# schwanbeck/YSMR

Measured on AMD Instinct MI355X. Metric: frames/sec detect+link, 1228x922 ~500 blobs, 1/2/4/8 GPU; HBM GB/s %peak, higher is better.
Workload: dtype u8 image / f32 threshold+geometry / f64 link; 1 GPU; 1228x922 stream, ~500 blobs, detect+link end to end (BASELINE configs[2], the configuration the metric is quoted on); detect_batch=248, channels=1, streams=1, parallelism=1 stream/GPU x1, tracks_alive=508, ids_issued=796

## Files before the change

ysmr_amd/csrc/detect_plan.h:

```cpp
#pragma once
#include <algorithm>
#include <cmath>
#include <cstddef>
#include <cstdint>

#include "hd.h"
#include "ysmr_hip.h"

namespace detect_plan {

constexpr int CU_COUNT = 256;
constexpr int TW = 64, TH = 32;
constexpr int STRIP_HALO_LANES = 3;
constexpr int STRIP_MAX_OUT_LANES = 64 - 2 * STRIP_HALO_LANES;
constexpr int STRIP_RESIDENT = 768;
#ifndef TM_MAX_PANEL_N
#define TM_MAX_PANEL_N 1232
#endif
#ifndef TM_START_ROWS_N
#define TM_START_ROWS_N 48
#endif
constexpr int TM_START_ROWS = TM_START_ROWS_N;
constexpr int TM_MAX_PANEL = TM_MAX_PANEL_N;

constexpr int NR_STRIDE = 32;
constexpr int SHARED_COUNTERS = 8;
constexpr int HOLED_CAP = 4096;
constexpr int WIN_CORE = 32;
#ifndef WIN_GROUP_N
#define WIN_GROUP_N 8
#endif
constexpr int WIN_GROUP = WIN_GROUP_N;
constexpr int CLEAR_BLOCKS = 512;
#ifndef WINDOW_BLOCKS_N
#define WINDOW_BLOCKS_N 1024
#endif
constexpr int WINDOW_BLOCKS = WINDOW_BLOCKS_N;
#ifndef WINDOW_BLOCKS_FREE_N
// ... 87 lines not shown
    return (cv_flavour & YSMR_BESIDE_BATCH_LINK) ? 248 : ((cv_flavour & YSMR_BESIDE_SPLIT_LINK) ? 160 : CU_COUNT);
}

inline bool mfma_supported(int H, int W, int channels, int t_low, int t_high, int use_high)
{
    const int gap = use_high ? (t_high > t_low ? t_high - t_low : t_low - t_high) : 1;
    return channels == 1 && (W & 3) == 0 && W >= 64 && W <= 16384 && H >= 18 && H <= 16383 && gap >= 1 &&
           t_low > -1000 && t_low < 1000 && t_high > -1000 && t_high < 1000;
}

struct StripShape {
    int out_lanes, strips_x, seg_h, segs_y;
    int by_xcd;
    unsigned blocks;
};
struct MfmaShape {
    int panels, panel_w;
    int by_xcd;
    int start_rows;
    unsigned grid;
};
enum class Kernel { refused, mfma, strip, tile };
struct ThresholdPlan {
    Kernel kernel;
    int mfma_variant;
    MfmaShape mfma;
    StripShape strip;
    unsigned tile_grid[3];
};

inline MfmaShape mfma_shape(int batch, int H, int W, int blocks_wanted, size_t mfma_lds)
{
    MfmaShape m{};
    m.panels = (W + TM_MAX_PANEL - 1) / TM_MAX_PANEL;
    m.panel_w = ((W + m.panels - 1) / m.panels + 15) & ~15;
    m.panels = (W + m.panel_w - 1) / m.panel_w;
    const int per_cu = (int)((160 * 1024) / mfma_lds);
    const int blocks = blocks_wanted * per_cu;
    const long long grid = std::max<long long>(1, std::min<long long>((long long)batch * m.panels * H / 32, blocks));
    m.by_xcd = (batch % 8 == 0 && grid % 8 == 0) ? 1 : 0;
    const long long groups = m.by_xcd ? 8 : 1, cols = (long long)(batch / groups) * m.panels, nb = grid / groups;
    m.start_rows = nb % cols == 0 ? 0 : TM_START_ROWS;
    m.grid = (unsigned)grid;
    return m;
}

inline StripShape strip_shape(int batch, int H, int W, const Knobs &kn)
{
    StripShape s{};
    const int quads = (W + 3) / 4;
    s.strips_x = (quads + STRIP_MAX_OUT_LANES - 1) / STRIP_MAX_OUT_LANES;
    s.out_lanes = (quads + s.strips_x - 1) / s.strips_x;
    const int resident = kn.thr_blocks > 0 ? kn.thr_blocks : STRIP_RESIDENT;
    const long long columns = (long long)batch * s.strips_x;
    const long long segs = std::max<long long>(1, (long long)resident * 4 / columns);
    s.seg_h = kn.seg_h > 0 ? kn.seg_h : (int)std::max<long long>(32, (H + segs - 1) / segs);
    s.segs_y = (H + s.seg_h - 1) / s.seg_h;
    const long long waves = columns * s.segs_y;
    long long blocks = std::min<long long>((waves + 3) / 4, resident);
    s.by_xcd = (batch % 8 == 0 && blocks % 8 == 0) ? 1 : 0;
    if (s.by_xcd && blocks / 8 * 4 > (long long)(batch / 8) * s.strips_x * s.segs_y)
        blocks = (((long long)(batch / 8) * s.strips_x * s.segs_y + 3) / 4) * 8;
    s.blocks = (unsigned)blocks;
    return s;
}

inline ThresholdPlan threshold_plan(int batch, int H, int W, int channels, int t_low, int t_high, int use_high, int cv_flavour,
                                    int variant, const Knobs &kn, size_t mfma_lds)
{
    ThresholdPlan p{};
    if (variant == 0 && (cv_flavour & YSMR_BESIDE_LINK)) variant = 1;
    if (variant != 1 && mfma_supported(H, W, channels, t_low, t_high, use_high)) {
        p.kernel = Kernel::mfma;
        p.mfma_variant = variant >= 2 ? variant - 1 : 0;
        p.mfma = mfma_shape(batch, H, W, kn.thr_blocks > 0 ? kn.thr_blocks : threshold_workgroups(cv_flavour), mfma_lds);
        return p;
    }
    if (variant >= 2) return p;
    const int t_gap = use_high ? (t_high > t_low ? t_high - t_low : t_low - t_high) : 0;
    if ((W & 3) == 0 && W >= 16 && H >= 2 && t_low > -100000 && t_low < 100000 && t_high > -100000 && t_high < 100000 && t_gap <= 127) {
        p.kernel = Kernel::strip;
        p.strip = strip_shape(batch, H, W, kn);
    } else {
        p.kernel = Kernel::tile;
        p.tile_grid[0] = (unsigned)((W + TW - 1) / TW); p.tile_grid[1] = (unsigned)((H + TH - 1) / TH); p.tile_grid[2] = (unsigned)batch;
    }
    return p;
// ... 151 lines not shown
```

ysmr_amd/csrc/thr_mfma.h:

```cpp
#pragma once
#include <hip/hip_runtime.h>
#include <cstdint>
#include "detect_plan.h"

namespace ysmr_thr {

struct Params {
    int H, W, batch;
    int panels, panel_w;
    int by_xcd;
    int inv, use_high, t_low, t_high;
    float neg_x_mul, k_first, d2;
    float col_scale, row_scale;
    uint32_t sh1, k1, sh2, k2;
    int start_rows;
    float kw[6];
};

size_t lds_bytes();

int launch(hipStream_t st, const uint8_t *frames, uint8_t *cls, int batch, int H, int W, int inv, int t_low, int t_high,
           int use_high, const float *gauss11, const detect_plan::MfmaShape &shape, int variant, hipEvent_t ev_start = nullptr,
           hipEvent_t ev_stop = nullptr);

}
```

ysmr_amd/csrc/thr_mfma.hip:

```cpp
#include "common.h"
#include "thr_mfma.h"
#include <cstring>
#include <mutex>
#include <type_traits>

namespace {

typedef _Float16 half8_t __attribute__((ext_vector_type(8)));
typedef _Float16 half2_t __attribute__((ext_vector_type(2)));
typedef float f32x4 __attribute__((ext_vector_type(4)));
typedef int i32x4 __attribute__((ext_vector_type(4)));
typedef uint32_t u32x4 __attribute__((ext_vector_type(4)));

#ifndef TM_MEM_WAVE_N
#define TM_MEM_WAVE_N 0
#endif
constexpr bool TM_MEM_WAVE = TM_MEM_WAVE_N != 0;
#ifndef TM_WAVES_N
#define TM_WAVES_N 16
#endif
constexpr int TM_WAVES = TM_WAVES_N, TM_THREADS = 64 * TM_WAVES;
constexpr int TM_ROWS = 16;
using detect_plan::TM_MAX_PANEL;
constexpr int TM_MAX_TILES = TM_MAX_PANEL / 16;
// ... 27 lines not shown
#define TM_STORE_AT_START_N 1
#endif
constexpr bool TM_STORE_AT_START = TM_STORE_AT_START_N != 0;
#ifndef TM_BLUR_GROUP_N
#define TM_BLUR_GROUP_N 1
#endif
constexpr int TM_BLUR_GROUP = TM_BLUR_GROUP_N;
#ifndef TM_PREFETCH_N
#define TM_PREFETCH_N 1
#endif
constexpr bool TM_PREFETCH = TM_PREFETCH_N != 0;
#ifndef TM_LIST_CAP_N
#define TM_LIST_CAP_N 248
#endif
constexpr int TM_LIST_CAP = TM_LIST_CAP_N;

#ifdef YSMR_STAMPS
constexpr int TM_ST_STEPS = 20, TM_ST_N = 8;
__device__ unsigned long long g_tm_stamps[TM_WAVES][TM_ST_STEPS][TM_ST_N];
#define TMSTAMP(step, k) do { if (blockIdx.x == TM_ST_BLOCK && (step) < TM_ST_STEPS && lane == 0) g_tm_stamps[wave][step][k] = __builtin_amdgcn_s_memtime(); } while (0)
#ifndef TM_ST_BLOCK
#define TM_ST_BLOCK 100
#endif
#else
#define TMSTAMP(step, k) do {} while (0)
#endif

__device__ __forceinline__ int opaque_lane(int lane) { asm volatile("" : "+v"(lane)); return lane; }

struct ThrItem {
    int f, x0, x1, y0, y1;
};

__device__ __forceinline__ int reflect101(int i, int n) { if (i < 0) i = -i; if (i >= n) i = 2 * (n - 1) - i; return i; }
__device__ __forceinline__ int clampi(int v, int lo, int hi) { return v < lo ? lo : (v > hi ? hi : v); }

__device__ __forceinline__ float sub_f16_lo(float x, uint32_t h)
{
    float r;
    asm("v_fma_mix_f32 %0, %1, -1.0, %2 op_sel_hi:[1,0,0]" : "=v"(r) : "v"(h), "v"(x));
    return r;
}
__device__ __forceinline__ float sub_f16_hi(float x, uint32_t h)
{
    float r;
    asm("v_fma_mix_f32 %0, %1, -1.0, %2 op_sel:[1,0,0] op_sel_hi:[1,0,0]" : "=v"(r) : "v"(h), "v"(x));
    return r;
// ... 46 lines not shown
    __builtin_amdgcn_wave_barrier();
    __builtin_amdgcn_fence(__ATOMIC_ACQUIRE, "wavefront");
    const int yy = clampi(y - 5 + min(dy, 10), 0, H - 1);
    const int ra = reflect101(yy - 1, H) - (y - 6), rb = yy - (y - 6), rc = reflect101(yy + 1, H) - (y - 6);
    float acc = 0.0f;
    uint32_t centre = 0;
#pragma unroll 1
    for (int i = 0; i < 11; ++i) {
        const int xx = clampi(x - 5 + i, 0, W - 1);
        const int ca = reflect101(xx - 1, W) - (x - 6), cb = xx - (x - 6), cc = reflect101(xx + 1, W) - (x - 6);
        const uint32_t s = win[16 * ra + ca] + 2u * win[16 * ra + cb] + win[16 * ra + cc] +
                           2u * (win[16 * rb + ca] + 2u * win[16 * rb + cb] + win[16 * rb + cc]) +
                           win[16 * rc + ca] + 2u * win[16 * rc + cb] + win[16 * rc + cc];
        const uint32_t b = (s + 8u) >> 4;
        if (i == 5) centre = b;
        acc = __builtin_fmaf((float)b, tap_weight(P, i), acc);
    }
    float m = __builtin_fmaf(__shfl(acc, base + 5, 64), P.kw[5], 0.0f);
#pragma unroll 1
    for (int j = 1; j <= 5; ++j) m = __builtin_fmaf(__shfl(acc, base + 5 + j, 64) + __shfl(acc, base + 5 - j, 64), P.kw[5 - j], m);
    const uint32_t s = (uint32_t)__shfl((int)centre, base + 5, 64);
    const int mi = clampi((int)__builtin_rintf(m), 0, 255);
    const int d = (int)s - mi;
    const int lo = P.inv ? (d <= P.t_low) : (d > P.t_low);
    const int hi = P.use_high ? (P.inv ? (d <= P.t_high) : (d > P.t_high)) : lo;
    return (uint32_t)(lo | (hi << 1));
}

__device__ __forceinline__ uint32_t exact_class_wave(const uint8_t *frame, const ysmr_thr::Params &P, int y, int x, int lane, uint8_t *scratch)
{
    const int H = P.H, W = P.W;
    uint8_t *win = scratch;
    float *bl = reinterpret_cast<float *>(scratch + 208);
    uint8_t g[3];
#pragma unroll
// ... 18 lines not shown
        const uint32_t sum = win[16 * ra + ca] + 2u * win[16 * ra + cb] + win[16 * ra + cc] +
                             2u * (win[16 * rb + ca] + 2u * win[16 * rb + cb] + win[16 * rb + cc]) +
                             win[16 * rc + ca] + 2u * win[16 * rc + cb] + win[16 * rc + cc];
        bl[12 * dy + i] = (float)((sum + 8u) >> 4);
    }
    __builtin_amdgcn_fence(__ATOMIC_RELEASE, "wavefront");
    __builtin_amdgcn_wave_barrier();
    __builtin_amdgcn_fence(__ATOMIC_ACQUIRE, "wavefront");
    const float *row = bl + 12 * min(lane, 10);
    float v[11];
#pragma unroll
    for (int i = 0; i < 11; ++i) v[i] = row[i];
    const float centre = bl[12 * 5 + 5];
    float acc = 0.0f;
#pragma unroll
    for (int i = 0; i < 11; ++i) acc = __builtin_fmaf(v[i], tap_weight(P, i), acc);
    auto at = [&](int l) { return __builtin_bit_cast(float, __builtin_amdgcn_readlane(__builtin_bit_cast(int, acc), l)); };
    float m = __builtin_fmaf(at(5), P.kw[5], 0.0f);
#pragma unroll
    for (int j = 1; j <= 5; ++j) m = __builtin_fmaf(at(5 + j) + at(5 - j), P.kw[5 - j], m);
    const int mi = clampi((int)__builtin_rintf(m), 0, 255);
    const int d = (int)centre - mi;
    const int lo = P.inv ? (d <= P.t_low) : (d > P.t_low);
    const int hi = P.use_high ? (P.inv ? (d <= P.t_high) : (d > P.t_high)) : lo;
    return (uint32_t)(lo | (hi << 1));
}

struct Lds {
    _Float16 tile[TM_PLANES ? 4 * TM_POS * 8 : TM_POS * TM_COL_PITCH];
    __device__ __forceinline__ _Float16 *at(int pos, int row)
    {
        return TM_PLANES ? &tile[(row >> 3) * (TM_POS * 8) + pos * 8 + (row & 7)] : &tile[pos * TM_COL_PITCH + row];
    }
    uint8_t raw[2][TM_ROWS * TM_RAW_PITCH];
    uint32_t out[TM_WAVES][TM_MEM_WAVE ? TM_ROWS * 16 * TM_MAX_TILES / 4 / TM_WAVES : TM_ROWS * TM_OUT_PITCH / 4];
    uint8_t side[TM_MEM_WAVE ? 2 : 1][512];
    uint32_t list[TM_LIST_CAP];
    uint16_t list_f[TM_LIST_CAP];
    uint32_t n_list;
};
static_assert(sizeof(Lds) <= 160 * 1024, "LDS of one CU");
static_assert(!TM_MEM_WAVE || (TM_ROWS * 16 * TM_MAX_TILES / 4) % TM_WAVES == 0, "the dense staging rows as TM_WAVES equal parts");
static_assert(sizeof(Lds::out) >= 256 * (TM_THREADS / 16), "the exact path's windows live in the class-byte staging");
static_assert(sizeof(Lds::out) >= 768 * TM_WAVES, "and so does the wave-per-pixel form's scratch");

__device__ __forceinline__ uint32_t small_f16(int w) { return w == 0 ? 0u : w == 1 ? 0x2C00u : w == 2 ? 0x3000u : w == 3 ? 0x3200u : 0x3400u; }

template <int EPS_MODE>
__global__ __launch_bounds__(TM_THREADS) __attribute__((amdgpu_waves_per_eu(4, 4))) void k_threshold_mfma(const uint8_t *__restrict__ frames, uint8_t *__restrict__ cls,
                                                               ysmr_thr::Params P)
{
    extern __shared__ __align__(16) uint8_t lds_bytes[];
    Lds &L = *reinterpret_cast<Lds *>(lds_bytes);
    const int tid = threadIdx.x, lane = tid & 63;
    const int wave = __builtin_amdgcn_readfirstlane(tid >> 6);
    const int H = P.H, W = P.W;
    const int l16 = lane & 15, q = lane >> 4;

    uint32_t thi[4];
    uint32_t tv[4];
    uint32_t tbh[4];
    uint32_t thh[4];
    uint32_t bid[4];
#pragma unroll
    for (int jj = 0; jj < 4; ++jj) {
        uint32_t b1 = 0;
#pragma unroll
        for (int e = 0; e < 4; ++e) {
            const int d = 16 * q + 4 * jj + e - 16 - l16;
            b1 |= (uint32_t)(d == 0 ? 2 : (d == 1 || d == -1) ? 1 : 0) << (8 * e);
        }
        thi[jj] = b1;
// ... 18 lines not shown
        }
        tv[jj] = v0; bid[jj] = bd;
        tbh[jj] = bh;
        thh[jj] = hh;
    }
    const i32x4 THI = {(int)thi[0], (int)thi[1], (int)thi[2], (int)thi[3]};
    i32x4 K_ROW = {0x6600, 0x6600, 0x6600, 0x6600};
    f32x4 K_COL = {768.5f, 768.5f, 768.5f, 768.5f};
    f32x4 K_LO = {P.k_first, P.k_first, P.k_first, P.k_first};
    asm volatile("" : "+v"(K_ROW), "+v"(K_COL), "+v"(K_LO));
    const half8_t BID = as_half8(bid[0], bid[1], bid[2], bid[3]);
    const half8_t TBh = as_half8(tbh[0], tbh[1], tbh[2], tbh[3]);

    for (int i = tid; i < (int)((sizeof(L.tile) + sizeof(L.raw)) / 4); i += TM_THREADS) reinterpret_cast<uint32_t *>(lds_bytes)[i] = 0u;
    if (tid == 0) L.n_list = 0;
    asm volatile("s_waitcnt lgkmcnt(0)\n\ts_barrier" ::: "memory");

    const int groups = P.by_xcd ? 8 : 1;
    const long long cols = (long long)(P.batch / groups) * P.panels, rows_all = cols * H;
    const long long nb = gridDim.x / groups, bi = P.by_xcd ? (blockIdx.x >> 3) : blockIdx.x;
    (void)rows_all;
    const long long vh = H + P.start_rows, v_all = cols * vh;
    auto real_row = [&](long long v) { const long long c = v / vh, r = v - c * vh; return c * H + (r > P.start_rows ? r - P.start_rows : 0); };
    long long g0 = real_row(v_all * bi / nb);
    const long long g1 = bi + 1 == nb ? cols * H : real_row(v_all * (bi + 1) / nb);
    const int f_add = P.by_xcd ? (int)(blockIdx.x & 7u) : 0;

    uint32_t n_kept = 0;
    while (g0 < g1) {
        ThrItem it;
        {
            const long long col = g0 / H;
            it.f = (int)(col / P.panels) * groups + f_add;
            const int panel = (int)(col % P.panels);
            it.x0 = panel * P.panel_w; it.x1 = min(it.x0 + P.panel_w, W);
            it.y0 = (int)(g0 % H);
            it.y1 = (int)min((long long)H, it.y0 + (g1 - g0));
            g0 += it.y1 - it.y0;
        }
        const uint8_t *frame = frames + (size_t)it.f * H * W;
        uint8_t *dst = cls + (size_t)it.f * H * W;
        const int PW = it.x1 - it.x0;
        int ntiles = (PW + 15) >> 4;
        const int nch = ntiles + 4;
        const int nblk = (it.y1 - it.y0 + TM_ROWS - 1) / TM_ROWS;
        const bool edge_l = it.x0 == 0, edge_r = it.x1 == W;
        int u0 = TM_MEM_WAVE ? 5 * wave + (wave > 3) + (wave > 7) + (wave > 11) : wave * TM_PER_WAVE;
        int cnt = TM_MEM_WAVE ? (wave == TM_WAVES - 1 ? 0 : 5 + ((wave & 3) == 3)) : TM_PER_WAVE;
        auto yb = [&](int j) { return it.y0 - 8 + TM_ROWS * j; };

        const int npieces = (TM_ROWS * nch + 63) >> 6;
        const uint32_t nch_recip = 65536u / (uint32_t)nch + 1u;
        const int part_c = lane < 16 ? 1 : (W - (it.x0 - 24)) >> 4;
        const int part_col = it.x0 - 24 + 16 * part_c;
        const bool part_lane = lane < 32 && part_c < nch && (lane < 16 ? edge_l : edge_r);
        auto part_load = [&](int j, u32x4 &v, uint32_t &last4) __attribute__((always_inline)) {
            const uint8_t *row = frame + (size_t)clampi(yb(j) + 1 + (lane & 15), 0, H - 1) * W;
#pragma unroll
            for (int i = 0; i < 4; ++i) v[i] = *reinterpret_cast<const uint32_t *>(row + clampi(part_col + 4 * i, 0, W - 4));
            last4 = *reinterpret_cast<const uint32_t *>(row + W - 4);
// ... 325 lines not shown
                        if (EPS_MODE == 2 || __builtin_amdgcn_ballot_w64(!calm) != 0ull) {
                            uint32_t f2 = (uint32_t)__builtin_amdgcn_cvt_pk_bf8_f32(c2[0] + P.d2, c2[1] + P.d2, 0, false);
                            f2 = (uint32_t)__builtin_amdgcn_cvt_pk_bf8_f32(c2[2] + P.d2, c2[3] + P.d2, (int)f2, true);
                            cb = ((f1 >> P.sh1) & P.k1) | ((f2 >> P.sh2) & P.k2);
                            uint32_t amb = ~(f1 & f2) & 0x40404040u;
                            if (EPS_MODE == 2) amb = 0x40404040u;
                            if (__builtin_expect(__builtin_amdgcn_ballot_w64(amb != 0u) != 0ull, 0)) {
                                const int lc = opaque_lane(lane), l16 = lc & 15, q = lc >> 4;
                                const int y = oy + l16;
                                if (amb != 0u && y < it.y1) {
#pragma unroll
                                    for (int r = 0; r < 4; ++r) {
                                        const int x = it.x0 + 16 * t + 4 * q + r;
                                        if (((amb >> (8 * r)) & 0xFFu) && x < it.x1) {
                                            const uint32_t slot = atomicAdd(&L.n_list, 1u);
                                            if (slot < (uint32_t)TM_LIST_CAP) { L.list[slot] = ((uint32_t)y << 16) | (uint32_t)x; L.list_f[slot] = (uint16_t)it.f; }
                                        }
                                    }
                                }
                            }
                        }
                        *reinterpret_cast<uint32_t *>(wout + 16 * ti) = cb;
                    }
                }
                if (bi == TM_DMA_AFTER_BLOCK && late_dma) mine = request_raw(s + 2);
                if (bi & 1) __builtin_amdgcn_sched_barrier(0);
            }
        };
        constexpr int ST_ITERS = TM_STORE_ROWS ? (TM_ROWS * TM_MAX_TILES + 64 * TM_WAVES - 1) / (64 * TM_WAVES) : (TM_ROWS * TM_PER_WAVE + 63) / 64;
        int st_lds[ST_ITERS], st_g[ST_ITERS];
        bool st_full[ST_ITERS], st_part[ST_ITERS];
// ... 145 lines not shown

        auto wait_all_but = [&](int n) __attribute__((always_inline)) {
            static_assert(TM_PIECES_PER_WAVE <= 3, "counted wait");
            if (n <= 0) asm volatile("s_waitcnt vmcnt(0)" ::: "memory");
            else if (n == 1) asm volatile("s_waitcnt vmcnt(1)" ::: "memory");
            else if (n == 2) asm volatile("s_waitcnt vmcnt(2)" ::: "memory");
            else asm volatile("s_waitcnt vmcnt(3)" ::: "memory");
        };
#if !defined(TM_PRIO_FLAT) && !defined(TM_PRIO4) && !defined(TM_PRIO4R)
        if (wave >= TM_WAVES / 2) __builtin_amdgcn_s_setprio(1);
#elif defined(TM_PRIO4)
        if ((wave >> 2) == 1) __builtin_amdgcn_s_setprio(1); else if ((wave >> 2) == 2) __builtin_amdgcn_s_setprio(2); else if ((wave >> 2) == 3) __builtin_amdgcn_s_setprio(3);
#elif defined(TM_PRIO4R)
        if ((wave >> 2) == 2) __builtin_amdgcn_s_setprio(1); else if ((wave >> 2) == 1) __builtin_amdgcn_s_setprio(2); else if ((wave >> 2) == 0) __builtin_amdgcn_s_setprio(3);
#endif
        request_raw(-1);
        request_raw(0);
        asm volatile("s_waitcnt vmcnt(0) lgkmcnt(0)\n\ts_barrier" ::: "memory");
        blur_step(-1, std::integral_constant<int, 1>{}, std::true_type{});
        asm volatile("s_waitcnt lgkmcnt(0)\n\ts_barrier" ::: "memory");
        if (nblk >= 1) request_raw(1);
        blur_any(0);
        asm volatile("s_waitcnt vmcnt(0) lgkmcnt(0)\n\ts_barrier" ::: "memory");
        if constexpr (TM_MEM_WAVE) {
            const bool is_mem = wave == TM_WAVES - 1;
#ifndef TM_MEM_PRIO_FLAT
            if (is_mem) __builtin_amdgcn_s_setprio(3);
#endif
            for (int s = 0; s <= nblk; ++s) {
                int n_dma = 0, unused = 0;
#ifndef TM_NO_FRESH
                asm volatile("" : "+s"(ntiles), "+s"(cnt), "+s"(u0));
#endif
                TMSTAMP(s, 0);
                if (is_mem && s + 2 <= nblk) n_dma = request_all(s + 2);
                TMSTAMP(s, 1);
                if (s >= 1 && cnt > 0) filter_step(s, false, unused);
                TMSTAMP(s, 2);
                if (is_mem) {
                    wait_all_but_n(n_dma);
                    if (s >= 1 && s + 1 <= nblk) side_patch(s + 1);
                }
                TMSTAMP(s, 3);
                TMSTAMP(s, 4);
                asm volatile("s_waitcnt lgkmcnt(0)\n\ts_barrier" ::: "memory");
                if (is_mem && s >= 1) store_rows(s);
                TMSTAMP(s, 5);
                if (s + 1 <= nblk && cnt > 0) blur_any(s + 1);
                TMSTAMP(s, 6);
                asm volatile("s_waitcnt lgkmcnt(0)\n\ts_barrier" ::: "memory");
                TMSTAMP(s, 7);
            }
        } else {
        for (int s = 0; s <= nblk; ++s) {
                int mine = 0;
                TMSTAMP(s, 0);
    #ifdef YSMR_STAMPS
                if (blockIdx.x == TM_ST_BLOCK && lane == 0 && wave == 0 && (s == 3 || s == 13)) {
                    unsigned long long rt;
                    asm volatile("s_memrealtime %0\n\ts_waitcnt lgkmcnt(0)" : "=s"(rt) :: "memory");
                    g_tm_stamps[1][s == 3 ? 18 : 19][0] = rt;
                    g_tm_stamps[1][s == 3 ? 18 : 19][1] = __builtin_amdgcn_s_memtime();
                }
    #endif
                if (!TM_STORE_ROWS && TM_STORE_AT_START && s >= 2) store_step(s - 1);
                const bool late_dma = TM_DMA_AFTER_BLOCK >= 0 && s >= 1 && s + 2 <= nblk && wave >= TM_WAVES / 2;
                if (s + 2 <= nblk && !late_dma) mine = request_raw(s + 2);
                TMSTAMP(s, 1);
                if (s >= 1) filter_step(s, late_dma, mine);
                TMSTAMP(s, 2);
                wait_all_but(__builtin_amdgcn_readfirstlane(mine));
                TMSTAMP(s, 3);
                if (!TM_STORE_ROWS && !TM_STORE_AT_START && s >= 1) store_step(s);
                TMSTAMP(s, 4);
                asm volatile("s_waitcnt lgkmcnt(0)\n\ts_barrier" ::: "memory");
                if (TM_STORE_ROWS && s >= 1) store_step(s);
                TMSTAMP(s, 5);
                if (s + 1 <= nblk) blur_any(s + 1);
                TMSTAMP(s, 6);
                asm volatile("s_waitcnt lgkmcnt(0)\n\ts_barrier" ::: "memory");
                TMSTAMP(s, 7);
            }
            if (!TM_STORE_ROWS && TM_STORE_AT_START && nblk >= 1) store_step(nblk);
    
        }

        const uint32_t n_now = L.n_list;
        if (__builtin_expect(n_now > (uint32_t)TM_LIST_CAP, 0)) {
            asm volatile("s_waitcnt vmcnt(0)\n\ts_barrier" ::: "memory");
            const int npx = PW * (it.y1 - it.y0);
            for (int p0 = 0; p0 < npx; p0 += TM_THREADS / 16) {
                const int p = min(p0 + (tid >> 4), npx - 1);
                const int y = it.y0 + p / PW, x = it.x0 + p % PW;
                const uint32_t c = exact_class(frame, P, y, x, lane, reinterpret_cast<uint8_t *>(L.out) + 256 * (tid >> 4));
                if (p0 + (tid >> 4) < npx && l16 == 0) dst[(size_t)y * W + x] = (uint8_t)c;
            }
            asm volatile("s_waitcnt vmcnt(0) lgkmcnt(0)\n\ts_barrier" ::: "memory");
            if (tid == 0) L.n_list = n_kept;
            asm volatile("s_waitcnt lgkmcnt(0)\n\ts_barrier" ::: "memory");
        } else n_kept = n_now;
    }

#ifdef TM_DBG_NOREFINE
    n_kept = 0;
#endif
    if (__builtin_expect(n_kept != 0u, 0)) {
        asm volatile("s_waitcnt vmcnt(0)\n\ts_barrier" ::: "memory");
        for (uint32_t e0 = 0; e0 < n_kept; e0 += TM_WAVES) {
            const uint32_t e = e0 + (uint32_t)wave;
            const uint32_t ent = L.list[min(e, n_kept - 1)];
            const size_t fo = (size_t)L.list_f[min(e, n_kept - 1)] * H * W;
            const int y = (int)(ent >> 16), x = (int)(ent & 0xFFFFu);
            const uint32_t c = exact_class_wave(frames + fo, P, y, x, lane, reinterpret_cast<uint8_t *>(L.out) + 768 * wave);
            if (e < n_kept && lane == 0) cls[fo + (size_t)y * W + x] = (uint8_t)c;
        }
    }
}

}

#ifdef YSMR_STAMPS
extern "C" int ysmr_debug_read_thr_stamps(unsigned long long *out) { return (int)hipMemcpyFromSymbol(out, HIP_SYMBOL(g_tm_stamps), sizeof(g_tm_stamps)); }
#endif

namespace ysmr_thr {

size_t lds_bytes() { return sizeof(Lds); }

int launch(hipStream_t st, const uint8_t *frames, uint8_t *cls, int batch, int H, int W, int inv, int t_low, int t_high,
           int use_high, const float *gauss11, const detect_plan::MfmaShape &shape, int variant, hipEvent_t ev_start, hipEvent_t ev_stop)
{
    if (shape.panel_w > TM_MAX_PANEL)
        return ysmr::fail(YSMR_ERR_ARG, "panels of %d columns, the matrix-pipe threshold kernel was built for %d", shape.panel_w, TM_MAX_PANEL);
    static std::mutex mu;
    static float key[6] = {0, 0, 0, 0, 0, 0};
    static detect_plan::Scales cached{0.0, 0.0, 0.0};
    detect_plan::Scales sc;
    {
        std::lock_guard<std::mutex> lk(mu);
        if (!(cached.S > 0.0 && !std::memcmp(key, gauss11, sizeof(key)))) {
            cached = detect_plan::choose_scales(gauss11);
            std::memcpy(key, gauss11, sizeof(key));
        }
        sc = cached;
    }
    if (!(sc.S > 0.0)) return ysmr::fail(YSMR_ERR_ARG, "the matrix-pipe threshold kernel found no admissible scale for these taps");
    const detect_plan::LevelConsts c = detect_plan::level_consts(sc, inv, t_low, t_high, use_high, variant);
    Params P{};
    P.H = H; P.W = W; P.batch = batch;
    P.panels = shape.panels; P.panel_w = shape.panel_w; P.by_xcd = shape.by_xcd; P.start_rows = shape.start_rows;
    P.inv = inv; P.use_high = use_high; P.t_low = t_low; P.t_high = use_high ? t_high : t_low;
    for (int i = 0; i < 6; ++i) P.kw[i] = gauss11[i];
    P.col_scale = c.col_scale; P.row_scale = c.row_scale;
    P.neg_x_mul = c.neg_x_mul; P.k_first = c.k_first; P.d2 = c.d2;
    P.sh1 = c.sh1; P.k1 = c.k1; P.sh2 = c.sh2; P.k2 = c.k2;
    auto kern = variant == 2 ? k_threshold_mfma<2> : k_threshold_mfma<0>;
    YSMR_HIP_CHECK(hipFuncSetAttribute(reinterpret_cast<const void *>(kern), hipFuncAttributeMaxDynamicSharedMemorySize, (int)sizeof(Lds)));
    ysmr::launch(kern, dim3(shape.grid), dim3(TM_THREADS), sizeof(Lds), st, ev_start, ev_stop, frames, cls, P);
    YSMR_LAUNCH_CHECK();
    return YSMR_OK;
}

}
```

ysmr_amd/csrc/track.hip:

```cpp
#include "common.h"
#include "set_order.h"
#include "tracker_plan.h"
#include <algorithm>
#include <cmath>
#include <cstdlib>
#include <cstring>
#include <vector>

struct DetGrid {
    const int *start;
    const int *items;
    const float *hdr;
    const float2 *xy;
};

namespace plan = tracker_plan;

struct ysmr_tracker {
    TrackerDev d;
    TrackerDev d1;
    int par = 0;
    plan::Config cfg;
    plan::Caps caps;
    int dims = 2;
// ... 1692 lines not shown
    if (ids) ids[i] = t.id[slot];
    if (xy) { xy[2 * i] = t.pos[slot]; xy[2 * i + 1] = t.pos[t.capacity + slot]; }
    if (gone) gone[i] = t.gone[t.gone_by_row ? i : slot];
}

__global__ void k_peek_third(TrackerDev t, const double *pos3, double *third)
{
    const int i = blockIdx.x * blockDim.x + threadIdx.x;
    if (i < *t.n_tracks) third[i] = pos3[t.order[i]];
}

}

int ysmr::fused_max_det() { return FUSED_MAX_DET; }

#ifndef BL_PAUSE_TICKS_N
#define BL_PAUSE_TICKS_N 1200
#endif
constexpr int BL_PAUSE_TICKS = BL_PAUSE_TICKS_N;
__global__ __launch_bounds__(64) void k_pause(int ticks)
{
    unsigned long long t0, t;
    asm volatile("s_memrealtime %0\n\ts_waitcnt lgkmcnt(0)" : "=s"(t0)::"memory");
    do {
        __builtin_amdgcn_s_sleep(8);
        asm volatile("s_memrealtime %0\n\ts_waitcnt lgkmcnt(0)" : "=s"(t)::"memory");
    } while (t - t0 < (unsigned long long)ticks);
}

extern "C" {

int ysmr_gsff_gains(double fps, int n_min, double n_max, int n_f, int32_t *n_i_out, double *gains_out)
{
    int n_i[YSMR_MAX_FILTERS];
    if (plan::Status s = plan::horizons(fps, n_min, n_max, n_f, n_i)) return plan_fail(s);
    if (!n_i_out) return ysmr::fail(YSMR_ERR_ARG, "n_i_out must not be NULL");
    size_t off = 0;
    for (int i = 0; i < n_f; ++i) {
        n_i_out[i] = n_i[i];
        if (gains_out) plan::closed_form_gain(n_i[i], gains_out + off);
        off += 4 * (size_t)n_i[i];
    }
    return YSMR_OK;
}
// ... 349 lines not shown
        for (int f0 = 0; f0 < batch; f0 += BL_MAX_BATCH) {
            const int nb = std::min(batch - f0, BL_MAX_BATCH);
            const float *det = det_dev + (size_t)f0 * md * 5;
            const double *third = d3 ? third_dev + (size_t)f0 * md : nullptr;
            int block = 2;
            for (int s = 0; s < 2; ++s) {
                const ysmr_tracker::Prepared &p = t->prepared[s];
                if (f0 == 0 && batch <= BL_MAX_BATCH && p.det == (const void *)det_dev && p.third == (const void *)third_dev &&
                    p.count == (const void *)det_count_dev && p.batch == batch) {
                    block = s;
                    t->prepared[s] = ysmr_tracker::Prepared();
                }
            }
            const BatchDev bd = batch_dev(t, block);
            if (block == 2) bin_batch(t, st, det, third, det_count_dev + f0, nb, bd);
            if (BL_PAUSE_TICKS > 0) hipLaunchKernelGGL(k_pause, dim3(1), dim3(64), 0, st, BL_PAUSE_TICKS);
            if (d3) {
                BlKernArgs3 ka;
                ka.t = t->d; ka.bd = bd; ka.det_all = det; ka.third_all = third; ka.det_count = det_count_dev + f0; ka.batch = nb;
                ka.frame0 = first_frame_index + f0; ka.rows = rows_dev; ka.rows_capacity = rows_capacity;
                ka.row_count = row_count_dev; ka.seat3 = t->seat3;
                hipLaunchKernelGGL(k_batch3, dim3(1), dim3(BL_THREADS), t->caps.batch3_lds, st, ka);
            } else {
                BlKernArgs ka;
                ka.t = t->d; ka.bd = bd; ka.det_all = det; ka.det_count = det_count_dev + f0; ka.batch = nb;
                ka.frame0 = first_frame_index + f0; ka.rows = rows_dev; ka.rows_capacity = rows_capacity;
                ka.row_count = row_count_dev; ka.gains = t->bgains_dev;
                for (int k = 0; k < 4; ++k) ka.hz[k] = (k == 0 || k < t->d.n_f) && k < BL_NF ? t->d.n_i[k] : 0x7FFFFFFF;
                hipLaunchKernelGGL(k_batch, dim3(1), dim3(BL_THREADS), t->caps.batch_lds, st, ka);
            }
            YSMR_LAUNCH_CHECK();
// ... 103 lines not shown
```

Before: 294,600 frames/s.

## Replace static row partition in MFMA threshold kernel with atomic band work-stealing

The MFMA threshold kernel no longer gives each block a fixed contiguous row range. Frames are cut into 128-row bands grouped into segments, and blocks claim bands through per-segment global atomic counters. A block that runs out scans for open segments and steals from them, and a claim issued partway through a band lets a block extend its current item without a refill. The counters sit in a per-stream ring and are reset by the last block to finish. The change also removes the artificial k_pause kernel that was launched before batch linking, which adds atomic traffic and extra barriers in exchange.

```diff
diff --git a/ysmr_amd/csrc/detect_plan.h b/ysmr_amd/csrc/detect_plan.h
--- a/ysmr_amd/csrc/detect_plan.h
+++ b/ysmr_amd/csrc/detect_plan.h
@@ -22,6 +22,14 @@
 #endif
 constexpr int TM_START_ROWS = TM_START_ROWS_N;
 constexpr int TM_MAX_PANEL = TM_MAX_PANEL_N;
+#ifndef TM_BAND_ROWS_N
+#define TM_BAND_ROWS_N 128
+#endif
+constexpr int TM_BAND_ROWS = TM_BAND_ROWS_N;
+static_assert(TM_BAND_ROWS >= 32 && TM_BAND_ROWS % 16 == 0, "whole 16-row steps, and a band no shorter than what starting an item re-filters");
+constexpr int TM_MAX_SEGS = 16384;
+constexpr int TM_COUNTER_RING = 4;
+constexpr int TM_COUNTER_BLOCK = TM_MAX_SEGS + 64;
 
 constexpr int NR_STRIDE = 32;
 constexpr int SHARED_COUNTERS = 8;
@@ -139,11 +147,45 @@
     int by_xcd;
     unsigned blocks;
 };
+struct BandPlan {
+    int band_rows, nbands, seg_bands, nseg;
+    int batch, cols, segs;
+};
+struct BandRows { int frame, panel, y0, y1; };
+YSMR_HD_FORCE int band_seg_count(const BandPlan &b, int sg)
+{
+    const int first = sg / b.cols * b.seg_bands;
+    return b.nbands - first < b.seg_bands ? b.nbands - first : b.seg_bands;
+}
+YSMR_HD_FORCE BandRows band_rows_of(const BandPlan &b, int sg, int k, int H)
+{
+    const int col = sg % b.cols, part = sg / b.cols;
+    BandRows r;
+    r.frame = col % b.batch; r.panel = col / b.batch;
+    r.y0 = (part * b.seg_bands + k) * b.band_rows;
+    r.y1 = r.y0 + b.band_rows < H ? r.y0 + b.band_rows : H;
+    return r;
+}
+inline BandPlan band_plan(int batch, int H, int panels, unsigned grid)
+{
+    BandPlan b{};
+    b.band_rows = TM_BAND_ROWS;
+    b.nbands = (H + b.band_rows - 1) / b.band_rows;
+    b.batch = batch;
+    b.cols = batch * panels;
+    int parts = std::max<long long>(1, std::min<long long>(b.nbands, (long long)grid / b.cols));
+    parts = std::max(1, std::min(parts, TM_MAX_SEGS / b.cols));
+    b.seg_bands = (b.nbands + parts - 1) / parts;
+    b.nseg = (b.nbands + b.seg_bands - 1) / b.seg_bands;
+    b.segs = (int)std::min<long long>((long long)b.cols * b.nseg, INT32_MAX);
+    return b;
+}
 struct MfmaShape {
     int panels, panel_w;
     int by_xcd;
     int start_rows;
     unsigned grid;
+    BandPlan bands;
 };
 enum class Kernel { refused, mfma, strip, tile };
 struct ThresholdPlan {
@@ -167,6 +209,7 @@
     const long long groups = m.by_xcd ? 8 : 1, cols = (long long)(batch / groups) * m.panels, nb = grid / groups;
     m.start_rows = nb % cols == 0 ? 0 : TM_START_ROWS;
     m.grid = (unsigned)grid;
+    m.bands = band_plan(batch, H, m.panels, m.grid);
     return m;
 }
 
@@ -195,7 +238,8 @@
 {
     ThresholdPlan p{};
     if (variant == 0 && (cv_flavour & YSMR_BESIDE_LINK)) variant = 1;
-    if (variant != 1 && mfma_supported(H, W, channels, t_low, t_high, use_high)) {
+    const bool mfma_batch = batch <= 65535 && (long long)batch * ((W + TM_MAX_PANEL - 1) / TM_MAX_PANEL) <= TM_MAX_SEGS;
+    if (variant != 1 && mfma_batch && mfma_supported(H, W, channels, t_low, t_high, use_high)) {
         p.kernel = Kernel::mfma;
         p.mfma_variant = variant >= 2 ? variant - 1 : 0;
         p.mfma = mfma_shape(batch, H, W, kn.thr_blocks > 0 ? kn.thr_blocks : threshold_workgroups(cv_flavour), mfma_lds);
diff --git a/ysmr_amd/csrc/thr_mfma.h b/ysmr_amd/csrc/thr_mfma.h
--- a/ysmr_amd/csrc/thr_mfma.h
+++ b/ysmr_amd/csrc/thr_mfma.h
@@ -8,12 +8,12 @@
 struct Params {
     int H, W, batch;
     int panels, panel_w;
-    int by_xcd;
+    detect_plan::BandPlan bands;
+    uint32_t *counters;
     int inv, use_high, t_low, t_high;
     float neg_x_mul, k_first, d2;
     float col_scale, row_scale;
     uint32_t sh1, k1, sh2, k2;
-    int start_rows;
     float kw[6];
 };
 
diff --git a/ysmr_amd/csrc/thr_mfma.hip b/ysmr_amd/csrc/thr_mfma.hip
--- a/ysmr_amd/csrc/thr_mfma.hip
+++ b/ysmr_amd/csrc/thr_mfma.hip
@@ -1,7 +1,10 @@
 #include "common.h"
 #include "thr_mfma.h"
+#include <cstddef>
 #include <cstring>
+#include <map>
 #include <mutex>
+#include <utility>
 #include <type_traits>
 
 namespace {
@@ -65,6 +68,7 @@
 #define TM_LIST_CAP_N 248
 #endif
 constexpr int TM_LIST_CAP = TM_LIST_CAP_N;
+constexpr int TM_CLAIM_TID = TM_THREADS - 64;
 
 #ifdef YSMR_STAMPS
 constexpr int TM_ST_STEPS = 20, TM_ST_N = 8;
@@ -82,6 +86,37 @@
 struct ThrItem {
     int f, x0, x1, y0, y1;
 };
+
+struct ThrKernArgs {
+    const uint8_t *frames;
+    uint8_t *cls;
+    ysmr_thr::Params P;
+};
+static_assert(offsetof(ThrKernArgs, P) == 16 && alignof(ysmr_thr::Params) == 8, "k_threshold_mfma(frames, cls, P) as the segment holds it");
+typedef const __attribute__((address_space(4))) ThrKernArgs *ThrKernArgsPtr;
+__device__ __forceinline__ ThrKernArgsPtr thr_kernargs()
+{
+    ThrKernArgsPtr p = (ThrKernArgsPtr)__builtin_amdgcn_kernarg_segment_ptr();
+    asm volatile("" : "+s"(p));
+    return p;
+}
+__device__ __forceinline__ detect_plan::BandPlan thr_bands()
+{
+    ThrKernArgsPtr a = thr_kernargs();
+    detect_plan::BandPlan b;
+    b.band_rows = a->P.bands.band_rows; b.nbands = a->P.bands.nbands; b.seg_bands = a->P.bands.seg_bands; b.nseg = a->P.bands.nseg;
+    b.batch = a->P.bands.batch; b.cols = a->P.bands.cols; b.segs = a->P.bands.segs;
+    return b;
+}
+__device__ __forceinline__ ysmr_thr::Params thr_exact_params()
+{
+    ThrKernArgsPtr a = thr_kernargs();
+    ysmr_thr::Params P;
+    P.H = a->P.H; P.W = a->P.W;
+    P.inv = a->P.inv; P.use_high = a->P.use_high; P.t_low = a->P.t_low; P.t_high = a->P.t_high;
+    return P;
+}
+__device__ __forceinline__ float thr_kw(int i) { return thr_kernargs()->P.kw[i]; }
 
 __device__ __forceinline__ int reflect101(int i, int n) { if (i < 0) i = -i; if (i >= n) i = 2 * (n - 1) - i; return i; }
 __device__ __forceinline__ int clampi(int v, int lo, int hi) { return v < lo ? lo : (v > hi ? hi : v); }
@@ -158,11 +193,11 @@
                            win[16 * rc + ca] + 2u * win[16 * rc + cb] + win[16 * rc + cc];
         const uint32_t b = (s + 8u) >> 4;
         if (i == 5) centre = b;
-        acc = __builtin_fmaf((float)b, tap_weight(P, i), acc);
+        acc = __builtin_fmaf((float)b, thr_kw(i <= 5 ? i : 10 - i), acc);
     }
-    float m = __builtin_fmaf(__shfl(acc, base + 5, 64), P.kw[5], 0.0f);
+    float m = __builtin_fmaf(__shfl(acc, base + 5, 64), thr_kw(5), 0.0f);
 #pragma unroll 1
-    for (int j = 1; j <= 5; ++j) m = __builtin_fmaf(__shfl(acc, base + 5 + j, 64) + __shfl(acc, base + 5 - j, 64), P.kw[5 - j], m);
+    for (int j = 1; j <= 5; ++j) m = __builtin_fmaf(__shfl(acc, base + 5 + j, 64) + __shfl(acc, base + 5 - j, 64), thr_kw(5 - j), m);
     const uint32_t s = (uint32_t)__shfl((int)centre, base + 5, 64);
     const int mi = clampi((int)__builtin_rintf(m), 0, 255);
     const int d = (int)s - mi;
@@ -211,11 +246,11 @@
     const float centre = bl[12 * 5 + 5];
     float acc = 0.0f;
 #pragma unroll
-    for (int i = 0; i < 11; ++i) acc = __builtin_fmaf(v[i], tap_weight(P, i), acc);
+    for (int i = 0; i < 11; ++i) acc = __builtin_fmaf(v[i], thr_kw(i <= 5 ? i : 10 - i), acc);
     auto at = [&](int l) { return __builtin_bit_cast(float, __builtin_amdgcn_readlane(__builtin_bit_cast(int, acc), l)); };
-    float m = __builtin_fmaf(at(5), P.kw[5], 0.0f);
-#pragma unroll
-    for (int j = 1; j <= 5; ++j) m = __builtin_fmaf(at(5 + j) + at(5 - j), P.kw[5 - j], m);
+    float m = __builtin_fmaf(at(5), thr_kw(5), 0.0f);
+#pragma unroll
+    for (int j = 1; j <= 5; ++j) m = __builtin_fmaf(at(5 + j) + at(5 - j), thr_kw(5 - j), m);
     const int mi = clampi((int)__builtin_rintf(m), 0, 255);
     const int d = (int)centre - mi;
     const int lo = P.inv ? (d <= P.t_low) : (d > P.t_low);
@@ -235,6 +270,7 @@
     uint32_t list[TM_LIST_CAP];
     uint16_t list_f[TM_LIST_CAP];
     uint32_t n_list;
+    uint32_t claim_walk, claim_item, open_seg;
 };
 static_assert(sizeof(Lds) <= 160 * 1024, "LDS of one CU");
 static_assert(!TM_MEM_WAVE || (TM_ROWS * 16 * TM_MAX_TILES / 4) % TM_WAVES == 0, "the dense staging rows as TM_WAVES equal parts");
@@ -253,6 +289,14 @@
     const int wave = __builtin_amdgcn_readfirstlane(tid >> 6);
     const int H = P.H, W = P.W;
     const int l16 = lane & 15, q = lane >> 4;
+
+    auto counters = [&]() -> uint32_t * { return thr_kernargs()->P.counters + 1; };
+    auto n_segs = [&]() -> uint32_t { return (uint32_t)thr_kernargs()->P.bands.segs; };
+    auto home_seg = [&]() -> uint32_t { return (uint32_t)__builtin_amdgcn_readfirstlane((int)(blockIdx.x % n_segs())); };
+    uint32_t first_claim = 0;
+    if (tid == TM_CLAIM_TID) first_claim = atomicAdd(counters() + home_seg(), 1u);
+    auto tid_late = [&]() -> int { return wave * 64 + lane; };
+    auto claim_thread = [&]() -> bool { return wave == TM_WAVES - 1 && lane == 0; };
 
     uint32_t thi[4];
     uint32_t tv[4];
@@ -301,36 +345,58 @@
 
     for (int i = tid; i < (int)((sizeof(L.tile) + sizeof(L.raw)) / 4); i += TM_THREADS) reinterpret_cast<uint32_t *>(lds_bytes)[i] = 0u;
     if (tid == 0) L.n_list = 0;
+    if (tid == TM_CLAIM_TID) L.claim_item = first_claim;
     asm volatile("s_waitcnt lgkmcnt(0)\n\ts_barrier" ::: "memory");
 
-    const int groups = P.by_xcd ? 8 : 1;
-    const long long cols = (long long)(P.batch / groups) * P.panels, rows_all = cols * H;
-    const long long nb = gridDim.x / groups, bi = P.by_xcd ? (blockIdx.x >> 3) : blockIdx.x;
-    (void)rows_all;
-    const long long vh = H + P.start_rows, v_all = cols * vh;
-    auto real_row = [&](long long v) { const long long c = v / vh, r = v - c * vh; return c * H + (r > P.start_rows ? r - P.start_rows : 0); };
-    long long g0 = real_row(v_all * bi / nb);
-    const long long g1 = bi + 1 == nb ? cols * H : real_row(v_all * (bi + 1) / nb);
-    const int f_add = P.by_xcd ? (int)(blockIdx.x & 7u) : 0;
+    auto seg_bands_uniform = [&](uint32_t sg) -> uint32_t { return (uint32_t)__builtin_amdgcn_readfirstlane(detect_plan::band_seg_count(thr_bands(), (int)sg)); };
+    auto claim_between = [&](uint32_t sg) -> uint32_t {
+        __syncthreads();
+        if (claim_thread()) L.claim_item = atomicAdd(counters() + sg, 1u);
+        __syncthreads();
+        return (uint32_t)__builtin_amdgcn_readfirstlane((int)__hip_atomic_load(&L.claim_item, __ATOMIC_RELAXED, __HIP_MEMORY_SCOPE_WORKGROUP));
+    };
+    auto look = [&]() -> uint32_t {
+        __syncthreads();
+        if (tid_late() == 0) L.open_seg = 0xFFFFFFFFu;
+        __syncthreads();
+        const detect_plan::BandPlan bands = thr_bands();
+        const uint32_t nsegs = (uint32_t)bands.segs, home = home_seg();
+        const uint32_t *ctr = counters();
+        for (uint32_t i = (uint32_t)tid_late(); i < nsegs; i += TM_THREADS)
+            if (__hip_atomic_load(&ctr[i], __ATOMIC_RELAXED, __HIP_MEMORY_SCOPE_AGENT) < (uint32_t)detect_plan::band_seg_count(bands, (int)i))
+                atomicMin(&L.open_seg, i >= home ? i - home : i + nsegs - home);
+        __syncthreads();
+        const uint32_t d = (uint32_t)__builtin_amdgcn_readfirstlane((int)__hip_atomic_load(&L.open_seg, __ATOMIC_RELAXED, __HIP_MEMORY_SCOPE_WORKGROUP));
+        return d == 0xFFFFFFFFu ? nsegs : (home + d >= nsegs ? home + d - nsegs : home + d);
+    };
 
     uint32_t n_kept = 0;
-    while (g0 < g1) {
+    uint32_t seg = home_seg(), seg_n = seg_bands_uniform(seg);
+    uint32_t k = (uint32_t)__builtin_amdgcn_readfirstlane((int)__hip_atomic_load(&L.claim_item, __ATOMIC_RELAXED, __HIP_MEMORY_SCOPE_WORKGROUP));
+    for (;;) {
+        if (k >= seg_n) {
+            seg = look();
+            if (seg >= n_segs()) break;
+            seg_n = seg_bands_uniform(seg);
+            k = claim_between(seg);
+            continue;
+        }
         ThrItem it;
         {
-            const long long col = g0 / H;
-            it.f = (int)(col / P.panels) * groups + f_add;
-            const int panel = (int)(col % P.panels);
-            it.x0 = panel * P.panel_w; it.x1 = min(it.x0 + P.panel_w, W);
-            it.y0 = (int)(g0 % H);
-            it.y1 = (int)min((long long)H, it.y0 + (g1 - g0));
-            g0 += it.y1 - it.y0;
+            const detect_plan::BandRows r = detect_plan::band_rows_of(thr_bands(), (int)seg, (int)k, H);
+            it.f = __builtin_amdgcn_readfirstlane(r.frame);
+            const int panel_w = thr_kernargs()->P.panel_w;
+            it.x0 = __builtin_amdgcn_readfirstlane(r.panel) * panel_w; it.x1 = min(it.x0 + panel_w, W);
+            it.y0 = __builtin_amdgcn_readfirstlane(r.y0); it.y1 = __builtin_amdgcn_readfirstlane(r.y1);
         }
+        constexpr uint32_t NO_CLAIM = 0xFFFFFFFFu, CLAIM_INFLIGHT = 0xFFFFFFFEu;
+        uint32_t k_last = k, k_next = NO_CLAIM;
         const uint8_t *frame = frames + (size_t)it.f * H * W;
         uint8_t *dst = cls + (size_t)it.f * H * W;
         const int PW = it.x1 - it.x0;
         int ntiles = (PW + 15) >> 4;
         const int nch = ntiles + 4;
-        const int nblk = (it.y1 - it.y0 + TM_ROWS - 1) / TM_ROWS;
+        int nblk = (it.y1 - it.y0 + TM_ROWS - 1) / TM_ROWS;
         const bool edge_l = it.x0 == 0, edge_r = it.x1 == W;
         int u0 = TM_MEM_WAVE ? 5 * wave + (wave > 3) + (wave > 7) + (wave > 11) : wave * TM_PER_WAVE;
         int cnt = TM_MEM_WAVE ? (wave == TM_WAVES - 1 ? 0 : 5 + ((wave & 3) == 3)) : TM_PER_WAVE;
@@ -686,7 +752,7 @@
                                         const int x = it.x0 + 16 * t + 4 * q + r;
                                         if (((amb >> (8 * r)) & 0xFFu) && x < it.x1) {
                                             const uint32_t slot = atomicAdd(&L.n_list, 1u);
-                                            if (slot < (uint32_t)TM_LIST_CAP) { L.list[slot] = ((uint32_t)y << 16) | (uint32_t)x; L.list_f[slot] = (uint16_t)it.f; }
+                                            if (slot < (uint32_t)TM_LIST_CAP) { L.list[slot] = ((uint32_t)y << 16) | (uint32_t)x; L.list_f[slot] = (uint16_t)opaque_lane(it.f); }
                                         }
                                     }
                                 }
@@ -862,6 +928,39 @@
 #elif defined(TM_PRIO4R)
         if ((wave >> 2) == 2) __builtin_amdgcn_s_setprio(1); else if ((wave >> 2) == 1) __builtin_amdgcn_s_setprio(2); else if ((wave >> 2) == 0) __builtin_amdgcn_s_setprio(3);
 #endif
+        auto claim_read = [&](int s) __attribute__((always_inline)) {
+            nblk = __builtin_amdgcn_readfirstlane(nblk); it.y1 = __builtin_amdgcn_readfirstlane(it.y1);
+            k_last = (uint32_t)__builtin_amdgcn_readfirstlane((int)k_last); k_next = (uint32_t)__builtin_amdgcn_readfirstlane((int)k_next);
+            asm volatile("" : "+s"(nblk), "+s"(it.y1), "+s"(k_last), "+s"(k_next));
+            if (k_next == CLAIM_INFLIGHT && s == nblk - 1) {
+                k_next = NO_CLAIM;
+                const uint32_t got = (uint32_t)__builtin_amdgcn_readfirstlane((int)__hip_atomic_load(&L.claim_walk, __ATOMIC_RELAXED, __HIP_MEMORY_SCOPE_WORKGROUP));
+                if (got == k_last + 1u && got < seg_n) {
+                    k_last = got;
+                    it.y1 = min(H, it.y1 + thr_kernargs()->P.bands.band_rows);
+                    nblk = (it.y1 - it.y0 + TM_ROWS - 1) / TM_ROWS;
+                } else k_next = got;
+            }
+        };
+        auto claim_issue = [&](int s, uint32_t &got) __attribute__((always_inline)) -> bool {
+            const bool now = k_next == NO_CLAIM && s == nblk - 2 && k_last + 1u < seg_n;
+            if (now && wave == TM_WAVES - 1) {
+                uint32_t *addr = counters() + seg;
+                uint64_t saved;
+                asm volatile("s_mov_b64 %0, exec\n\ts_mov_b64 exec, 1\n\tglobal_atomic_add %1, %2, %3, off sc0\n\ts_mov_b64 exec, %0"
+                             : "=&s"(saved), "+v"(got) : "v"(addr), "v"(1u) : "memory");
+            }
+            return now;
+        };
+        auto claim_publish = [&](bool now, uint32_t &got) __attribute__((always_inline)) {
+            if (now) {
+                if (wave == TM_WAVES - 1) {
+                    asm volatile("s_waitcnt vmcnt(0)" : "+v"(got) : : "memory");
+                    if (lane == 0) L.claim_walk = got;
+                }
+                k_next = CLAIM_INFLIGHT;
+            }
+        };
         request_raw(-1);
         request_raw(0);
         asm volatile("s_waitcnt vmcnt(0) lgkmcnt(0)\n\ts_barrier" ::: "memory");
@@ -877,6 +976,7 @@
 #endif
             for (int s = 0; s <= nblk; ++s) {
                 int n_dma = 0, unused = 0;
+                claim_read(s);
 #ifndef TM_NO_FRESH
                 asm volatile("" : "+s"(ntiles), "+s"(cnt), "+s"(u0));
 #endif
@@ -894,7 +994,10 @@
                 asm volatile("s_waitcnt lgkmcnt(0)\n\ts_barrier" ::: "memory");
                 if (is_mem && s >= 1) store_rows(s);
                 TMSTAMP(s, 5);
+                uint32_t claimed = 0;
+                const bool claim_now = claim_issue(s, claimed);
                 if (s + 1 <= nblk && cnt > 0) blur_any(s + 1);
+                claim_publish(claim_now, claimed);
                 TMSTAMP(s, 6);
                 asm volatile("s_waitcnt lgkmcnt(0)\n\ts_barrier" ::: "memory");
                 TMSTAMP(s, 7);
@@ -902,6 +1005,7 @@
         } else {
         for (int s = 0; s <= nblk; ++s) {
                 int mine = 0;
+                claim_read(s);
                 TMSTAMP(s, 0);
     #ifdef YSMR_STAMPS
                 if (blockIdx.x == TM_ST_BLOCK && lane == 0 && wave == 0 && (s == 3 || s == 13)) {
@@ -924,7 +1028,10 @@
                 asm volatile("s_waitcnt lgkmcnt(0)\n\ts_barrier" ::: "memory");
                 if (TM_STORE_ROWS && s >= 1) store_step(s);
                 TMSTAMP(s, 5);
+                uint32_t claimed = 0;
+                const bool claim_now = claim_issue(s, claimed);
                 if (s + 1 <= nblk) blur_any(s + 1);
+                claim_publish(claim_now, claimed);
                 TMSTAMP(s, 6);
                 asm volatile("s_waitcnt lgkmcnt(0)\n\ts_barrier" ::: "memory");
                 TMSTAMP(s, 7);
@@ -937,16 +1044,31 @@
         if (__builtin_expect(n_now > (uint32_t)TM_LIST_CAP, 0)) {
             asm volatile("s_waitcnt vmcnt(0)\n\ts_barrier" ::: "memory");
             const int npx = PW * (it.y1 - it.y0);
+            const ysmr_thr::Params PX = thr_exact_params();
+            const int tc = opaque_lane(tid_late()), lc = tc & 63;
             for (int p0 = 0; p0 < npx; p0 += TM_THREADS / 16) {
-                const int p = min(p0 + (tid >> 4), npx - 1);
+                const int p = min(p0 + (tc >> 4), npx - 1);
                 const int y = it.y0 + p / PW, x = it.x0 + p % PW;
-                const uint32_t c = exact_class(frame, P, y, x, lane, reinterpret_cast<uint8_t *>(L.out) + 256 * (tid >> 4));
-                if (p0 + (tid >> 4) < npx && l16 == 0) dst[(size_t)y * W + x] = (uint8_t)c;
+                const uint32_t c = exact_class(frame, PX, y, x, lc, reinterpret_cast<uint8_t *>(L.out) + 256 * (tc >> 4));
+                if (p0 + (tc >> 4) < npx && (lc & 15) == 0) dst[(size_t)y * W + x] = (uint8_t)c;
             }
             asm volatile("s_waitcnt vmcnt(0) lgkmcnt(0)\n\ts_barrier" ::: "memory");
-            if (tid == 0) L.n_list = n_kept;
+            if (tid_late() == 0) L.n_list = n_kept;
             asm volatile("s_waitcnt lgkmcnt(0)\n\ts_barrier" ::: "memory");
         } else n_kept = n_now;
+        k = k_next < CLAIM_INFLIGHT ? k_next : (k_last + 1u < seg_n ? claim_between(seg) : seg_n);
+    }
+    if (wave == 0) {
+        uint32_t last = 0;
+        if (lane == 0) {
+            __threadfence();
+            last = atomicAdd(thr_kernargs()->P.counters, 1u) + 1u == gridDim.x ? 1u : 0u;
+        }
+        if (__builtin_amdgcn_readfirstlane((int)last)) {
+            __threadfence();
+            uint32_t *block = thr_kernargs()->P.counters;
+            for (uint32_t i = (uint32_t)lane, n = n_segs(); i <= n; i += 64u) __hip_atomic_store(&block[i], 0u, __ATOMIC_RELAXED, __HIP_MEMORY_SCOPE_AGENT);
+        }
     }
 
 #ifdef TM_DBG_NOREFINE
@@ -954,12 +1076,13 @@
 #endif
     if (__builtin_expect(n_kept != 0u, 0)) {
         asm volatile("s_waitcnt vmcnt(0)\n\ts_barrier" ::: "memory");
+        const ysmr_thr::Params PX = thr_exact_params();
         for (uint32_t e0 = 0; e0 < n_kept; e0 += TM_WAVES) {
             const uint32_t e = e0 + (uint32_t)wave;
             const uint32_t ent = L.list[min(e, n_kept - 1)];
             const size_t fo = (size_t)L.list_f[min(e, n_kept - 1)] * H * W;
             const int y = (int)(ent >> 16), x = (int)(ent & 0xFFFFu);
-            const uint32_t c = exact_class_wave(frames + fo, P, y, x, lane, reinterpret_cast<uint8_t *>(L.out) + 768 * wave);
+            const uint32_t c = exact_class_wave(frames + fo, PX, y, x, lane, reinterpret_cast<uint8_t *>(L.out) + 768 * wave);
             if (e < n_kept && lane == 0) cls[fo + (size_t)y * W + x] = (uint8_t)c;
         }
     }
@@ -974,6 +1097,28 @@
 namespace ysmr_thr {
 
 size_t lds_bytes() { return sizeof(Lds); }
+
+static int counters_for(hipStream_t st, uint32_t **out)
+{
+    struct Ring { uint32_t *base; unsigned next; };
+    static std::mutex mu;
+    static std::map<std::pair<int, hipStream_t>, Ring> rings;
+    int dev = 0;
+    YSMR_HIP_CHECK(hipGetDevice(&dev));
+    std::lock_guard<std::mutex> lk(mu);
+    auto it = rings.find({dev, st});
+    if (it == rings.end()) {
+        const size_t bytes = sizeof(uint32_t) * detect_plan::TM_COUNTER_BLOCK * detect_plan::TM_COUNTER_RING;
+        uint32_t *base = nullptr;
+        YSMR_HIP_CHECK(hipMalloc(reinterpret_cast<void **>(&base), bytes));
+        const hipError_t e = hipMemsetAsync(base, 0, bytes, st);
+        if (e != hipSuccess) { (void)hipFree(base); YSMR_HIP_CHECK(e); }
+        it = rings.emplace(std::make_pair(dev, st), Ring{base, 0u}).first;
+    }
+    Ring &r = it->second;
+    *out = r.base + (size_t)(r.next++ % detect_plan::TM_COUNTER_RING) * detect_plan::TM_COUNTER_BLOCK;
+    return YSMR_OK;
+}
 
 int launch(hipStream_t st, const uint8_t *frames, uint8_t *cls, int batch, int H, int W, int inv, int t_low, int t_high,
            int use_high, const float *gauss11, const detect_plan::MfmaShape &shape, int variant, hipEvent_t ev_start, hipEvent_t ev_stop)
@@ -996,7 +1141,12 @@
     const detect_plan::LevelConsts c = detect_plan::level_consts(sc, inv, t_low, t_high, use_high, variant);
     Params P{};
     P.H = H; P.W = W; P.batch = batch;
-    P.panels = shape.panels; P.panel_w = shape.panel_w; P.by_xcd = shape.by_xcd; P.start_rows = shape.start_rows;
+    P.panels = shape.panels; P.panel_w = shape.panel_w;
+    const detect_plan::BandPlan &bands = shape.bands;
+    if (bands.segs < 1 || bands.segs > detect_plan::TM_MAX_SEGS || batch > 65535)
+        return ysmr::fail(YSMR_ERR_ARG, "%d row segments, the matrix-pipe threshold kernel has counters for %d", bands.segs, detect_plan::TM_MAX_SEGS);
+    P.bands = bands;
+    if (const int e = counters_for(st, &P.counters)) return e;
     P.inv = inv; P.use_high = use_high; P.t_low = t_low; P.t_high = use_high ? t_high : t_low;
     for (int i = 0; i < 6; ++i) P.kw[i] = gauss11[i];
     P.col_scale = c.col_scale; P.row_scale = c.row_scale;
diff --git a/ysmr_amd/csrc/track.hip b/ysmr_amd/csrc/track.hip
--- a/ysmr_amd/csrc/track.hip
+++ b/ysmr_amd/csrc/track.hip
@@ -1730,20 +1730,6 @@
 
 int ysmr::fused_max_det() { return FUSED_MAX_DET; }
 
-#ifndef BL_PAUSE_TICKS_N
-#define BL_PAUSE_TICKS_N 1200
-#endif
-constexpr int BL_PAUSE_TICKS = BL_PAUSE_TICKS_N;
-__global__ __launch_bounds__(64) void k_pause(int ticks)
-{
-    unsigned long long t0, t;
-    asm volatile("s_memrealtime %0\n\ts_waitcnt lgkmcnt(0)" : "=s"(t0)::"memory");
-    do {
-        __builtin_amdgcn_s_sleep(8);
-        asm volatile("s_memrealtime %0\n\ts_waitcnt lgkmcnt(0)" : "=s"(t)::"memory");
-    } while (t - t0 < (unsigned long long)ticks);
-}
-
 extern "C" {
 
 int ysmr_gsff_gains(double fps, int n_min, double n_max, int n_f, int32_t *n_i_out, double *gains_out)
@@ -2123,7 +2109,6 @@
             }
             const BatchDev bd = batch_dev(t, block);
             if (block == 2) bin_batch(t, st, det, third, det_count_dev + f0, nb, bd);
-            if (BL_PAUSE_TICKS > 0) hipLaunchKernelGGL(k_pause, dim3(1), dim3(64), 0, st, BL_PAUSE_TICKS);
             if (d3) {
                 BlKernArgs3 ka;
                 ka.t = t->d; ka.bd = bd; ka.det_all = det; ka.third_all = third; ka.det_count = det_count_dev + f0; ka.batch = nb;
```

Result: no change. 293,900 frames/s (-0.2%).
